# learner-shx/SVG-IR

Hardware: AMD Instinct MI355X
Metric: Gaussian-surfels/sec fwd+bwd @800x800 (1 view) (higher is better)
Workload: dtype f32; 1 GPU; cfg2: rgss path, P=200000 surfels, 800x800, SH degree 3, S=5, VS=0, fwd+bwd, one view per step per GPU (BASELINE.json configs[1] = cfg2 at N=1; configs[3] = cfg4, view r on rank r, at N>1); num_rendered=673008, parallelism=view-parallel x1, per_rank_cpus=not pinned

## Files before the change

svg-ir_amd/csrc/api.hip:

```cpp
#include <algorithm>
#include <cstdarg>
#include <cstdio>
#include <atomic>
#include <cstdlib>
#include <ctime>
#include <memory>
#include <mutex>
#include <string>
#include <vector>

#include "common.hpp"
#include "workload_history.hpp"

using namespace svgir;

namespace {

thread_local std::string g_err;
std::atomic<bool> g_prof{false};
WorkloadHistory g_history;
unsigned long long* pinned_words(size_t n) {
    void* ptr = nullptr;
    if (hipHostMalloc(&ptr, n * sizeof(unsigned long long), hipHostMallocCoherent) != hipSuccess) { (void)hipGetLastError(); return nullptr; }
    std::fill_n((unsigned long long*)ptr, n, 0ull);
    return (unsigned long long*)ptr;
}
unsigned long long* g_pinned = nullptr;
std::atomic<uint32_t> g_pinned_tag{0};
constexpr unsigned kPinnedSlots = 256;
std::once_flag g_pinned_once;
std::mutex g_pinned_mu;
uint64_t g_pinned_busy[kPinnedSlots / 64];
struct PinnedSlot {
    unsigned long long* at = nullptr; uint32_t tag = 0; int index = -1;
    PinnedSlot() {
        std::call_once(g_pinned_once, [] { g_pinned = pinned_words(2 * kPinnedSlots); });
        tag = ++g_pinned_tag;
        if (tag == 0) tag = ++g_pinned_tag;
        if (!g_pinned) return;
        static const unsigned usable = [] { const char* e = getenv("SVGIR_PINNED_SLOTS"); return e ? (unsigned)std::min<long>(std::max<long>(atol(e), 0), kPinnedSlots) : kPinnedSlots; }();
        std::lock_guard<std::mutex> lk(g_pinned_mu);
        for (unsigned i = 0; i < usable; i++)
            if (!(g_pinned_busy[i / 64] >> (i % 64) & 1ull)) {
                g_pinned_busy[i / 64] |= 1ull << (i % 64);
                index = (int)i;
                at = g_pinned + 2 * index;
                return;
            }
    }
    ~PinnedSlot() {
        if (index < 0) return;
        std::lock_guard<std::mutex> lk(g_pinned_mu);
        g_pinned_busy[index / 64] &= ~(1ull << (index % 64));
    }
    PinnedSlot(const PinnedSlot&) = delete;
    PinnedSlot& operator=(const PinnedSlot&) = delete;
};
double spin_budget_s() {
    static const double v = [] {
        const char* e = getenv("SVGIR_SPIN_MS");
        return e ? std::max(0.0, atof(e)) * 1e-3 : 0.05;
    }();
    return v;
}
// ... 252 lines not shown
        if (p->variant != SVGIR_SVGSS) return fail(SVGIR_ERR_INVALID, "fused shading belongs to the svgss variant");
        if (sp.P != p->P) return fail(SVGIR_ERR_INVALID, "fused shading: sp.P = %d but P = %d", sp.P, p->P);
        if (p->S != (sp.training ? 4 : 7) || p->VS != (sp.training ? 52 : 64))
            return fail(SVGIR_ERR_INVALID, "fused shading packs S = %d, VS = %d (training = %d), not S = %d, VS = %d", sp.training ? 4 : 7,
                        sp.training ? 52 : 64, sp.training, p->S, p->VS);
        if (!sp.viewmatrix) return fail(SVGIR_ERR_INVALID, "fused shading needs sp.viewmatrix (packed view-space normals)");
    }
    return 0;
}

CapKey workload_key(const svgir_params* p) {
    int dev_id = 0;
    (void)hipGetDevice(&dev_id);
    return CapKey{dev_id, p->W, p->H, p->P, p->S, p->variant == SVGIR_SVGSS ? p->VS : 0, p->variant, p->workload_scope};
}

bool bin_capacity(size_t bytes, const char* image_blob, int W, int H, int nstate, Wait how, const hipStream_t* stream, ViewCounts* vc) {
    const bool compact = bin_bytes_compact(bytes);
    if (compact || how != Wait::kCaps)
        *vc = resolve_view(image_blob, image_layout(const_cast<char*>(image_blob), W, H).counters, how, stream, compact);
    if (compact) return vc->known && vc->cap_slots >= 0;
    vc->cap_R = binning_capacity_from_bytes(bytes, view_grid(W, H).T, nstate);
    vc->cap_slots = -1;
    return true;
}

template <class A> void camera_args(A& a, const svgir_params* p) {
    a.P = p->P; a.D = p->D; a.M = p->M; a.means3D = p->means3D; a.shs = p->colors_precomp ? nullptr : p->shs;
    a.scales = p->scales; a.rotations = p->rotations; a.view = p->viewmatrix; a.proj = p->projmatrix; a.campos = p->cam_pos;
    a.scale_modifier = p->scale_modifier; a.tanx = p->tan_fovx; a.tany = p->tan_fovy; a.cfg = cfg_ref(p);
    a.focal_x = p->W / (2.0f * p->tan_fovx); a.focal_y = p->H / (2.0f * p->tan_fovy);
}

RenderArgs render_args(const svgir_params* p, const ViewGrid& v, const GeomLayout& G, const ImageLayout& I, const BinLayout& B, int fin) {
    const bool svgss = p->variant == SVGIR_SVGSS;
    RenderArgs ra{};
    ra.W = v.W; ra.H = v.H; ra.gx = v.gx; ra.gy = v.gy; ra.S = p->S; ra.VS = svgss ? p->VS : 0;
    ra.ranges = I.ranges; ra.point_list = B.val[fin]; ra.rec = G.rec; ra.features = p->features; ra.vfeatures = p->vfeatures;
    ra.bg = p->background; ra.cfg = cfg_ref(p);
    ra.sub_list = B.sub_list; ra.sub_total = I.sub_total; ra.sub_order = I.sub_order; ra.sub_count = I.sub_count; ra.sub_ndump = I.sub_ndump;
    ra.sub_pair_base = I.sub_pair_base; ra.sub_slot_base = I.sub_slot_base;
    ra.seg_list = B.seg_list; ra.seg_desc = B.seg_desc; ra.seg_count = I.counters; ra.seg_block = I.seg_block; ra.seg_state = B.seg_state;
    ra.slot_cap = (uint32_t)std::min<size_t>(B.slot_cap, 0xffffffffu);
    ra.order_n = (int)order_entries(v.gx, v.gy);
    ra.bg_in_render = render_specialised(p->S, ra.VS, svgss) ? 1 : 0;
    ra.final_T = I.final_T; ra.final_D = I.final_D; ra.n_contrib = I.n_contrib;
    return ra;
}
}

extern "C" {

int svgir_abi_version(void) { return SVGIR_ABI_VERSION; }
size_t svgir_geom_bytes(int32_t P) { return geom_layout(nullptr, P).bytes; }
size_t svgir_image_bytes(int32_t W, int32_t H) { return image_layout(nullptr, W, H).bytes; }
size_t svgir_binning_bytes(int32_t R, int32_t W, int32_t H, int32_t S, int32_t VS) {
    return bin_layout(nullptr, binning_capacity(R), view_grid(W, H).T, seg_nstate(S, VS)).bytes;
}
size_t svgir_image_ncontrib_offset(int32_t W, int32_t H) { return image_layout(nullptr, W, H).ncontrib_off; }
size_t svgir_image_ranges_offset(int32_t W, int32_t H) {
    const ImageLayout I = image_layout((char*)256, W, H);
    return (size_t)((char*)I.ranges - (char*)256);
}
size_t svgir_binning_point_list_offset(size_t binning_bytes, const char* image_blob, int32_t W, int32_t H, int32_t S, int32_t VS) {
    const int T = view_grid(W, H).T, nstate = seg_nstate(S, VS);
    ViewCounts vc;
    if (!bin_capacity(binning_bytes, image_blob, W, H, nstate, Wait::kCaps, nullptr, &vc)) return (size_t)-1;
    const BinLayout B = bin_layout((char*)256, vc.cap_R, T, nstate);
    return (size_t)((char*)B.val[tile_sort_plan(T).passes & 1] - (char*)256);
}
const char* svgir_last_error(void) { return g_err.c_str(); }
void svgir_set_profiling(int enabled) {
    resolve_pending();
    if (enabled) {
        std::lock_guard<std::mutex> lk(g_times_mu);
        g_accum.clear();
    }
    g_prof.store(enabled != 0);
}
int svgir_last_timings(const char** names, float* avg_ms, int* counts, int cap) {
    resolve_pending();
    std::lock_guard<std::mutex> lk(g_times_mu);
    int n = 0;
    for (auto& acc : g_accum) {
        if (n >= cap) break;
        names[n] = acc.name;
        avg_ms[n] = (float)(acc.sum_ms / (acc.count > 0 ? acc.count : 1));
        if (counts) counts[n] = acc.count;
        n++;
    }
    return n;
}

struct ForwardCall {
    const svgir_view_call c; const svgir_params* p = c.params; const svgir_outputs* o = c.outputs; hipStream_t s = (hipStream_t)c.stream;
    bool key_spec;
    int P = 0, nstate = 0, fin = 0, spec_top = -1, cap = 0;
    ViewGrid v{};
    bool svgss = false, shade_subset = false, prepass = false, done = false;
    char *gblob = nullptr, *iblob = nullptr, *bblob = nullptr;
    GeomLayout G{}; ImageLayout I{}; TileSortPlan plan{};
    CapKey ckey{}; const uint32_t* depth_order = nullptr; long long cap_slots = -1;
    hipEvent_t features_ready = nullptr;
    PinnedSlot R_pin;
    StageMarks tm;

    ForwardCall(const svgir_view_call& c_, bool key_spec_) : c(c_), key_spec(key_spec_), tm(stage_begin(s)) {}

    int check(const char* what) {
        hipError_t e = p->debug ? hipStreamSynchronize(s) : hipSuccess;
        if (e == hipSuccess) e = hipGetLastError();
        return e != hipSuccess ? fail(SVGIR_ERR_HIP, p->debug ? "%s failed: %s" : "%s launch failed: %s", what, hipGetErrorString(e)) : 0;
    }

    int run_binning_and_render(char* bblob, int cap, long long cap_slots, bool timed, bool cull_only = false) {
        const BinLayout B = bin_layout(bblob, cap, v.T, nstate, cap_slots);
        launch_emit(P, depth_order, G.tiles, G.offsets, G.rec, o->radii, v.gx, v.gy, B.key[0], B.val[0], cap, I.ranges,
                    I.counters, B.radix_tbl, G.counters + 3, s);
        if (int rc = check("emit")) return rc;
        if (timed) stage_mark(tm, "emit");
        if (plan.single) {
            launch_tile_sort12(B.key, B.val, cap, G.counters, B.radix_tbl, I.ranges, v.T, s);
            if (int rc = check("tile sort")) return rc;
            if (timed) stage_mark(tm, "sort_tile");
        } else {
            launch_radix_sort(B.key, B.val, cap, G.counters, plan.bits, plan.bits_per_pass, B.radix_tbl, s);
            if (int rc = check("tile sort")) return rc;
            if (timed) stage_mark(tm, "sort_tile");
            launch_ranges(cap, G.counters, B.key[fin], I.ranges, v.T, s);
            if (int rc = check("ranges")) return rc;
            if (timed) stage_mark(tm, "ranges");
        }

        RenderArgs ra = render_args(p, v, G, I, B, fin);
        ra.hi_fill = high_fill(g_history.guess_fill(ckey)) ? 1 : 0;
        ra.out_color = o->out_color; ra.out_normal = o->out_normal; ra.out_depth = o->out_depth; ra.out_opacity = o->out_opacity;
        ra.out_feature = o->out_feature; ra.out_vfeature = o->out_vfeature; ra.out_weights = o->out_weights;
        const bool clear_stencil = !svgss && !p->computer_pseudo_normal;
        ra.zero_a = clear_stencil ? o->out_pseudo_normal : nullptr;
        ra.zero_b = clear_stencil ? o->out_surface_xyz : nullptr;
        launch_cull(ra, s);
        uint32_t vtag = 0;
        unsigned long long* vslot = view_note(iblob, cap, cap_slots, &vtag, s);
        const bool row_path = svgss && p->VS > 0 && render_specialised(p->S, p->VS, true);
        static const int xcd_forced = [] { const char* e = getenv("SVGIR_FWD_XCD"); return e ? (atoi(e) != 0 ? 1 : 0) : -1; }();
        const bool per_xcd = ra.bg_in_render && (xcd_forced >= 0 ? xcd_forced != 0 : ra.hi_fill != 0);
        launch_order_desc(I.sub_total, 4 * v.T, I.sub_order, row_path ? I.sub_pair_base : nullptr, I.sub_slot_base, I.counters, vslot, vtag,
                          (uint32_t)cap, cap_slots, kBlobMagic, v.gx, ra.order_n, per_xcd, s);
        if (int rc = check("cull")) return rc;
        if (timed) stage_mark(tm, "cull");
        if (cull_only) return 0;
        if (prepass) {
            RenderArgs rp = ra;
            rp.S = 0; rp.VS = 0; rp.features = nullptr; rp.vfeatures = nullptr; rp.needed = G.needed;
            launch_contrib_prepass(rp, s);
            if (int rc = check("prepass")) return rc;
            if (timed) stage_mark(tm, "prepass");
        }
        if (p->shade) {
            svgir_shade_params sp = p->shade->sp;
            sp.subset = nullptr; sp.subset_count = nullptr;
            if (prepass) {
                uint32_t* cnt = G.shade_work + partition_work_words(P) - 1;
                launch_partition(P, G.needed, nullptr, G.shade_list, G.shade_work, cnt, s);
                sp.subset = G.shade_list; sp.subset_count = cnt;
            } else if (shade_subset) {
                sp.subset = depth_order; sp.subset_count = G.counters + 3;
            }
            if (shade_forward_impl(&sp, p->shade->reduced, const_cast<float*>(p->features), const_cast<float*>(p->vfeatures), true, s) != 0)
                return fail(SVGIR_ERR_INVALID, "fused shading: svgir_shade_forward rejected its parameters");
            if (int rc = check("shade")) return rc;
            if (timed) stage_mark(tm, "shade");
        }
        if (features_ready && hipStreamWaitEvent(s, features_ready, 0) != hipSuccess) return fail(SVGIR_ERR_HIP, "waiting for the features event");
        if (launch_render_fwd(ra, svgss, s) < 0) launch_render_fwd_generic(ra, svgss, s);
        if (int rc = check("render")) return rc;
        if (timed) stage_mark(tm, "render");
        return 0;
    }

    int begin() {
        if (int rc = validate(p, true)) return rc;
        features_ready = (hipEvent_t)p->features_ready;
        if (!o || !c.geom || !c.binning || !c.image) return fail(SVGIR_ERR_INVALID, "outputs / allocators must be provided");
        P = p->P; v = view_grid(p->W, p->H);
        svgss = p->variant == SVGIR_SVGSS;
        if (P == 0) {
            const size_t N = (size_t)v.W * v.H;
            HIP_OK(hipMemsetAsync(o->out_color, 0, 3 * N * 4, s));
            HIP_OK(hipMemsetAsync(o->out_normal, 0, 3 * N * 4, s));
            HIP_OK(hipMemsetAsync(o->out_depth, 0, N * 4, s));
            HIP_OK(hipMemsetAsync(o->out_opacity, 0, N * 4, s));
            if (p->S) HIP_OK(hipMemsetAsync(o->out_feature, 0, (size_t)p->S * N * 4, s));
            if (svgss && p->VS) HIP_OK(hipMemsetAsync(o->out_vfeature, 0, (size_t)(p->VS / 4) * N * 4, s));
            if (!svgss && o->out_pseudo_normal) HIP_OK(hipMemsetAsync(o->out_pseudo_normal, 0, 3 * N * 4, s));
            if (!svgss && o->out_surface_xyz) HIP_OK(hipMemsetAsync(o->out_surface_xyz, 0, 3 * N * 4, s));
            done = true;
            return 1;
        }
        gblob = c.geom(geom_layout(nullptr, P).bytes, c.geom_ctx);
        iblob = c.image(image_layout(nullptr, v.W, v.H).bytes, c.image_ctx);
        if (!gblob || !iblob) return fail(SVGIR_ERR_ALLOC, "geometry/image blob allocation failed");
        G = geom_layout(gblob, P);
        I = image_layout(iblob, v.W, v.H);

        PreArgs pa;
        camera_args(pa, p);
        pa.W = v.W; pa.H = v.H; pa.gx = v.gx; pa.gy = v.gy; pa.colors_precomp = p->colors_precomp; pa.opacities = p->opacities;
        pa.cov3D_precomp = p->cov3D_precomp; pa.patchbbox = p->patchbbox;
        pa.rec = G.rec; pa.cov3D = G.cov3D; pa.clamped = G.clamped; pa.tiles = G.tiles; pa.key = G.key[0]; pa.idx = G.idx[0];
        pa.radii = o->radii;
        pa.out_weights = o->out_weights;
        pa.features = nullptr; pa.embed_S = 0;
        if (rec_embeds_features(p->S, svgss ? p->VS : 0)) {
            if (features_ready && hipStreamWaitEvent(s, features_ready, 0) != hipSuccess) return fail(SVGIR_ERR_HIP, "waiting for the features event");
            features_ready = nullptr; pa.features = p->features; pa.embed_S = p->S; }
        shade_subset = p->shade && !p->shade->all_surfels;
        prepass = shade_subset && shade_prepass(p->shade->sp.Ns);
        pa.needed = prepass ? G.needed : nullptr;
        pa.span = G.counters + 3;
        if (p->shade) pa.tabs = shade_tables(&p->shade->sp, nullptr, 0);
        pa.zero_words = radix_gtot(G.radix_tbl, P); pa.n_zero_words = (int)radix_gtot_words(P);
        ckey = workload_key(p);
        static const bool key_spec_env = getenv("SVGIR_NO_KEY_SPEC") == nullptr;
        spec_top = (key_spec && key_spec_env) ? g_history.guess_top(ckey) : -1;
        pa.spec_top = spec_top; pa.key_top = G.key_top;
        pa.prefilter_violation = nullptr;
        if (p->prefiltered) {
            HIP_OK(hipMemsetAsync(G.counters, 0, 16, s));
            pa.prefilter_violation = G.counters + 1;
        }
        launch_preprocess(pa, svgss, s);
        if (int rc = check("preprocess")) return rc;
        stage_mark(tm, "preprocess");

        const int depth_bits = spec_top >= 0 ? 24 : 32;
        depth_order = G.idx[(depth_bits / 8) & 1];
        launch_radix_sort(G.key, G.idx, P, nullptr, depth_bits, 8, G.radix_tbl, s);
        if (int rc = check("depth sort")) return rc;
        stage_mark(tm, "sort_depth");

        launch_offsets_scan(G.tiles, depth_order, G.offsets, G.scan_tmp, P, G.counters, G.key_top, (P + 63) / 64, pa.prefilter_violation,
                            R_pin.at, R_pin.tag, s);
        if (int rc = check("offsets scan")) return rc;
        stage_mark(tm, "scan");

        nstate = seg_nstate(p->S, svgss ? p->VS : 0);
        plan = tile_sort_plan(v.T);
        fin = plan.passes & 1;

        cap = 0; cap_slots = -1; bblob = nullptr;
        CapKey pkey = ckey;
        (void)resolve_view(g_history.last_view(ckey, &pkey.P), nullptr, Wait::kLook, nullptr, false, &pkey);
        long long gs = -1;
        if (const int guess = g_history.guess(ckey, &gs)) {
            cap = binning_capacity((long long)guess + guess / 8 + 1024);
            cap_slots = p->forward_only ? 0 : (gs < 0 ? -1 : std::min<long long>(gs + gs / 8 + 64, (long long)seg_capacity(cap, v.T)));
            bblob = c.binning(bin_layout(nullptr, cap, v.T, nstate, cap_slots).bytes, c.binning_ctx);
            if (bblob) {
                if (int rc = run_binning_and_render(bblob, cap, cap_slots, true)) return rc;
            } else {
                cap = 0;
            }
        }
        return 0;
    }

    static int run(const svgir_view_call& c, bool key_spec) {
        ForwardCall f(c, key_spec);
        const int rc = f.begin();
        return rc != 0 ? (rc < 0 ? rc : 0) : f.finish();
    }

    int finish() {
        if (done) return 0;
        done = true;
        uint32_t R_host = 0, R_aux = 0;
        bool have_R = R_pin.at && pinned_spin(R_pin.at, R_pin.tag, &R_host, &R_aux);
        if (!have_R) {
            const hipError_t e = hipStreamSynchronize(s);
            if (e != hipSuccess) return fail(SVGIR_ERR_HIP, "the forward failed on the device: %s", hipGetErrorString(e));
            have_R = R_pin.at && tagged_pair(R_pin.at, R_pin.tag, &R_host, &R_aux);
            if (!have_R) {
                uint32_t w[3] = {0, 0, 0};
                HIP_OK(hipMemcpy(w, G.counters, 12, hipMemcpyDeviceToHost));
                R_host = w[0]; R_aux = ((p->prefiltered && w[1]) ? 1u << 16 : 0u) | (w[2] & 0xffffu);
            }
        }
        if (p->prefiltered && (R_aux >> 16) != 0u) {
            (void)hipStreamSynchronize(s);
            return fail(SVGIR_ERR_INVALID, "Point is filtered although prefiltered is set. This shouldn't happen!");
        }
        if (R_host > 0x7ffff000u) return fail(SVGIR_ERR_INVALID, "instance count %u overflows int32", R_host);
        const int R = (int)R_host;
        {
            const uint32_t summary = R_aux & 0xffffu;
            if (key_spec) { g_history.record_top(ckey, summary); g_history.count(WorkloadHistory::kForwards); }
            if (spec_top >= 0) g_history.count(WorkloadHistory::kThreePass);
            const int av = (int)((summary >> 8) & 0xffu), ov = (int)(summary & 0xffu);
            if (spec_top >= 0 && !(av == 0xff && ov == 0) && (av != spec_top || ov != spec_top)) {
                HIP_OK(hipStreamSynchronize(s));
                g_history.count(WorkloadHistory::kRerunTop);
// ... 345 lines not shown
```

svg-ir_amd/csrc/binning.hip:

```cpp
#include <algorithm>

#include "common.hpp"

namespace svgir {

namespace {

constexpr int GS = 32;

template <int ITEMS>
__global__ void __launch_bounds__(BLOCK) radix_hist_kernel(const uint32_t* __restrict__ keys, int n_cap,
                                                           const uint32_t* __restrict__ n_dev, int bit_lo,
                                                           uint32_t mask, uint32_t* __restrict__ table,
                                                           uint32_t* __restrict__ gtot) {
    __shared__ uint32_t hist[256];
    const int n = n_dev ? (int)min((uint32_t)n_cap, n_dev[0]) : n_cap;
    hist[threadIdx.x] = 0;
    __syncthreads();
    const int base = blockIdx.x * (BLOCK * ITEMS);
    uint32_t k[ITEMS];
#pragma unroll
    for (int i = 0; i < ITEMS; i++) k[i] = keys[max(0, min(base + i * BLOCK + (int)threadIdx.x, n - 1))];
#pragma unroll
    for (int i = 0; i < ITEMS; i++) {
        const int e = base + i * BLOCK + threadIdx.x;
        if (e < n) atomicAdd(&hist[(k[i] >> bit_lo) & mask], 1u);
    }
    __syncthreads();
    const uint32_t c = hist[threadIdx.x];
    table[(size_t)blockIdx.x * 256 + threadIdx.x] = c;
    if (c) atomicAdd(&gtot[(size_t)(blockIdx.x / GS) * 256 + threadIdx.x], c);
}

template <int ITEMS>
__global__ void __launch_bounds__(BLOCK) radix_scatter_kernel(const uint32_t* __restrict__ kin,
                                                              const uint32_t* __restrict__ vin,
                                                              uint32_t* __restrict__ kout, uint32_t* __restrict__ vout,
                                                              int n_cap, const uint32_t* __restrict__ n_dev, int bit_lo, int nbits,
                                                              const uint32_t* __restrict__ table,
                                                              const uint32_t* __restrict__ gtot, int ngroups) {
    __shared__ uint32_t wcnt[4][256];
    __shared__ uint32_t wtot[4];
    const int t = threadIdx.x, lane = t & 63, wave = t >> 6;
    const uint32_t mask = (1u << nbits) - 1;
    const int n = n_dev ? (int)min((uint32_t)n_cap, n_dev[0]) : n_cap;
    const int base = blockIdx.x * (BLOCK * ITEMS) + wave * (64 * ITEMS);
    const unsigned long long lt_mask = (lane == 0) ? 0ull : (~0ull >> (64 - lane));
    uint32_t ks[ITEMS], vs[ITEMS], rk[ITEMS];
#pragma unroll
    for (int c = 0; c < ITEMS; c++) {
        const int e = base + c * 64 + lane;
        ks[c] = e < n ? kin[e] : 0u;
        vs[c] = e < n ? vin[e] : 0u;
    }
#pragma unroll
// ... 46 lines not shown
        uint32_t incl = bc;
#pragma unroll
        for (int d = 1; d < 64; d <<= 1) {
            const uint32_t o = __shfl_up(incl, d);
            if (lane >= d) incl += o;
        }
        __syncthreads();
        if (lane == 63) wtot[wave] = incl;
        __syncthreads();
        uint32_t woff = 0;
#pragma unroll
        for (int w = 0; w < 4; w++) woff += w < wave ? wtot[w] : 0u;
        const uint32_t bs = woff + incl - bc;
        bstart[t] = bs; gcur[t] = cursor;
        wcnt[0][t] = bs; wcnt[1][t] = bs + c0; wcnt[2][t] = bs + c0 + c1; wcnt[3][t] = bs + c0 + c1 + c2;
        __syncthreads();
#pragma unroll
        for (int c = 0; c < ITEMS; c++) {
            if (base + c * 64 + lane < n) {
                const uint32_t lp = wcnt[wave][(ks[c] >> bit_lo) & mask] + rk[c];
                sK[lp] = ks[c]; sV[lp] = vs[c];
            }
        }
        __syncthreads();
        const int nblk = min(BLOCK * ITEMS, n - (int)blockIdx.x * (BLOCK * ITEMS));
#pragma unroll
        for (int c = 0; c < ITEMS; c++) {
            const int i = c * BLOCK + t;
            if (i < nblk) {
                const uint32_t k = sK[i], d = (k >> bit_lo) & mask;
                const uint32_t pos = gcur[d] + ((uint32_t)i - bstart[d]);
                kout[pos] = k;
                vout[pos] = sV[i];
            }
        }
        return;
    }
    {
        const uint32_t c0 = wcnt[0][t], c1 = wcnt[1][t], c2 = wcnt[2][t];
        __syncthreads();
        wcnt[0][t] = cursor; wcnt[1][t] = cursor + c0; wcnt[2][t] = cursor + c0 + c1; wcnt[3][t] = cursor + c0 + c1 + c2;
    }
    __syncthreads();
#pragma unroll
    for (int c = 0; c < ITEMS; c++) {
        if (base + c * 64 + lane < n) {
            const uint32_t pos = wcnt[wave][(ks[c] >> bit_lo) & mask] + rk[c];
            kout[pos] = ks[c];
            vout[pos] = vs[c];
        }
    }
}

__global__ void __launch_bounds__(BLOCK) ts12_hist_kernel(const uint32_t* __restrict__ keys, int n_cap, const uint32_t* __restrict__ n_dev,
                                                          uint32_t* __restrict__ table, int nbins) {
    __shared__ uint32_t hist[TS12_BINS];
    const int n = n_dev ? (int)min((uint32_t)n_cap, n_dev[0]) : n_cap;
    const int t = threadIdx.x;
    for (int i = t; i < nbins; i += BLOCK) hist[i] = 0u;
    __syncthreads();
    const int base = blockIdx.x * TS12_KEYS;
    uint32_t k[TS12_KEYS / BLOCK];
#pragma unroll
    for (int i = 0; i < TS12_KEYS / BLOCK; i++) k[i] = keys[max(0, min(base + i * BLOCK + t, n - 1))];
#pragma unroll
    for (int i = 0; i < TS12_KEYS / BLOCK; i++)
        if (base + i * BLOCK + t < n) atomicAdd(&hist[k[i] & (TS12_BINS - 1)], 1u);
    __syncthreads();
    uint32_t* row = table + (size_t)blockIdx.x * nbins;
    for (int i = t; i < nbins; i += BLOCK) row[i] = hist[i];
}

__global__ void __launch_bounds__(BLOCK) ts12_colscan_kernel(uint32_t* __restrict__ table, int nb, uint32_t* __restrict__ totals, int nbins) {
    __shared__ uint32_t psum[16][17];
    const int col = threadIdx.x & 15, seg = threadIdx.x >> 4;
    const int d = blockIdx.x * 16 + col;
    const int rps = (nb + 15) / 16, r0 = min(nb, seg * rps), r1 = min(nb, r0 + rps);
    uint32_t* colp = table + d;
    uint32_t sum = 0;
    int r = r0;
    for (; r + 8 <= r1; r += 8) {
        uint32_t c[8];
#pragma unroll
        for (int j = 0; j < 8; j++) c[j] = colp[(size_t)(r + j) * nbins];
#pragma unroll
        for (int j = 0; j < 8; j++) sum += c[j];
    }
    for (; r < r1; r++) sum += colp[(size_t)r * nbins];
    psum[seg][col] = sum;
    __syncthreads();
    uint32_t run = 0, all = 0;
#pragma unroll
    for (int sg = 0; sg < 16; sg++) { const uint32_t v = psum[sg][col]; run += sg < seg ? v : 0u; all += v; }
    if (seg == 0) totals[d] = all;
    r = r0;
    for (; r + 8 <= r1; r += 8) {
        uint32_t c[8];
#pragma unroll
        for (int j = 0; j < 8; j++) c[j] = colp[(size_t)(r + j) * nbins];
#pragma unroll
        for (int j = 0; j < 8; j++) { colp[(size_t)(r + j) * nbins] = run; run += c[j]; }
    }
    for (; r < r1; r++) { const uint32_t c = colp[(size_t)r * nbins]; colp[(size_t)r * nbins] = run; run += c; }
}

__global__ void __launch_bounds__(BLOCK) ts12_scatter_kernel(const uint32_t* __restrict__ kin, const uint32_t* __restrict__ vin,
                                                             uint32_t* __restrict__ kout, uint32_t* __restrict__ vout, int n_cap,
                                                             const uint32_t* __restrict__ n_dev, const uint32_t* __restrict__ table,
                                                             const uint32_t* __restrict__ totals, uint32_t* __restrict__ ranges, int T, int nbins) {
    __shared__ uint32_t cur[TS12_BINS];
    __shared__ uint16_t wcnt[4][TS12_BINS];
    __shared__ uint32_t wtot[4];
    constexpr int PERMAX = TS12_BINS / BLOCK;
    constexpr int ROUNDS = TS12_KEYS / BLOCK;
    const int per = nbins / BLOCK;
    const int t = threadIdx.x, lane = t & 63, wave = t >> 6;
    const int n = n_dev ? (int)min((uint32_t)n_cap, n_dev[0]) : n_cap;
    const int base = blockIdx.x * TS12_KEYS + wave * (64 * ROUNDS);
    const unsigned long long lt_mask = (lane == 0) ? 0ull : (~0ull >> (64 - lane));
    uint32_t ks[ROUNDS], vs[ROUNDS];
    uint16_t rk[ROUNDS];
#pragma unroll
    for (int c = 0; c < ROUNDS; c++) {
        const int e = base + c * 64 + lane;
        ks[c] = e < n ? kin[e] : 0u;
        vs[c] = e < n ? vin[e] : 0u;
    }
    uint32_t tot[PERMAX], pre[PERMAX];
    {
        const uint32_t* tp = totals + t * per;
        const uint32_t* rp = table + (size_t)blockIdx.x * nbins + t * per;
#pragma unroll
        for (int j = 0; j < PERMAX; j++) { tot[j] = j < per ? tp[j] : 0u; pre[j] = j < per ? rp[j] : 0u; }
    }
    uint32_t sum = 0;
#pragma unroll
    for (int j = 0; j < PERMAX; j++) sum += tot[j];
    uint32_t incl = sum;
#pragma unroll
    for (int d = 1; d < 64; d <<= 1) {
        const uint32_t o = __shfl_up(incl, d);
        if (lane >= d) incl += o;
    }
    if (lane == 63) wtot[wave] = incl;
#pragma unroll
    for (int w = 0; w < 4; w++)
        for (int i = t; i < nbins / 2; i += BLOCK) reinterpret_cast<uint32_t*>(&wcnt[w][0])[i] = 0u;
    __syncthreads();
    uint32_t run = incl - sum;
#pragma unroll
    for (int w = 0; w < 4; w++) run += w < wave ? wtot[w] : 0u;
#pragma unroll
    for (int j = 0; j < PERMAX; j++) {
        if (j < per) {
            const int tile = t * per + j;
            cur[tile] = run + pre[j];
            if (blockIdx.x == 0 && tile < T) {
                ranges[2 * tile] = tot[j] ? run : 0u;
                ranges[2 * tile + 1] = tot[j] ? run + tot[j] : 0u;
            }
            run += tot[j];
        }
    }
#pragma unroll
    for (int c = 0; c < ROUNDS; c++) {
        const bool valid = base + c * 64 + lane < n;
        const uint32_t d = ks[c] & (TS12_BINS - 1);
        unsigned long long same = __ballot(valid);
#pragma unroll
        for (int b = 0; b < 12; b++) {
            const unsigned long long m = __ballot((d >> b) & 1u);
            same &= ((d >> b) & 1u) ? m : ~m;
        }
        const uint32_t in_round = (uint32_t)__popcll(same & lt_mask);
        const uint32_t prior = wcnt[wave][d];
        rk[c] = (uint16_t)(prior + in_round);
        if (valid && in_round == 0) wcnt[wave][d] = (uint16_t)(prior + (uint32_t)__popcll(same));
    }
    __syncthreads();
#pragma unroll
    for (int c = 0; c < ROUNDS; c++) {
        if (base + c * 64 + lane < n) {
            const uint32_t d = ks[c] & (TS12_BINS - 1);
            uint32_t pos = cur[d] + rk[c];
            if (wave > 0) pos += wcnt[0][d];
            if (wave > 1) pos += wcnt[1][d];
            if (wave > 2) pos += wcnt[2][d];
            kout[pos] = ks[c];
            vout[pos] = vs[c];
        }
    }
}

__device__ __forceinline__ uint32_t block_exclusive_scan_2048(uint32_t (&v)[8], uint32_t* wsum, uint32_t& total) {
    const int t = threadIdx.x, lane = t & 63, wave = t >> 6;
    uint32_t s = 0;
#pragma unroll
    for (int i = 0; i < 8; i++) s += v[i];
    uint32_t incl = s;
#pragma unroll
    for (int d = 1; d < 64; d <<= 1) {
        const uint32_t o = __shfl_up(incl, d);
        if (lane >= d) incl += o;
    }
    if (lane == 63) wsum[wave] = incl;
    __syncthreads();
    uint32_t woff = 0, tot = 0;
#pragma unroll
    for (int w = 0; w < 4; w++) { const uint32_t x = wsum[w]; if (w < wave) woff += x; tot += x; }
    total = tot;
    return woff + incl - s;
}

__global__ void __launch_bounds__(BLOCK) offsets_reduce_kernel(const uint32_t* __restrict__ tiles,
                                                               const uint32_t* __restrict__ order, int n,
                                                               uint32_t* __restrict__ counts_out,
                                                               uint32_t* __restrict__ block_sums,
                                                               const uint32_t* __restrict__ key_top, int n_key_top,
                                                               uint32_t* __restrict__ block_key) {
    __shared__ uint32_t wsum[4];
    if (threadIdx.x < 64) {
        const int j = blockIdx.x * (SCAN_BLOCK_ELEMS / 64) + (int)threadIdx.x;
        uint32_t kv = (threadIdx.x < SCAN_BLOCK_ELEMS / 64 && j < n_key_top) ? key_top[j] : 0xff00u;
#pragma unroll
        for (int d = 32; d >= 1; d >>= 1) { const uint32_t o = (uint32_t)__shfl_xor((int)kv, d); kv = (kv & o & 0xff00u) | ((kv | o) & 0xffu); }
        if (threadIdx.x == 0) block_key[blockIdx.x] = kv;
    }
    uint32_t v[8];
    const int base = blockIdx.x * SCAN_BLOCK_ELEMS + threadIdx.x * 8;
    uint32_t oi[8];
#pragma unroll
    for (int i = 0; i < 8; i++) oi[i] = order[min(base + i, n - 1)];
#pragma unroll
    for (int i = 0; i < 8; i++) v[i] = tiles[2 * oi[i]];
#pragma unroll
    for (int i = 0; i < 8; i++) v[i] = (base + i < n) ? v[i] : 0u;
    if (base + 8 <= n) {
        reinterpret_cast<uint4*>(counts_out + base)[0] = make_uint4(v[0], v[1], v[2], v[3]);
        reinterpret_cast<uint4*>(counts_out + base)[1] = make_uint4(v[4], v[5], v[6], v[7]);
    } else {
#pragma unroll
        for (int i = 0; i < 8; i++) if (base + i < n) counts_out[base + i] = v[i];
    }
// ... 345 lines not shown

void launch_order_desc(const uint32_t* counts, int n, uint32_t* order, uint32_t* prefix, uint32_t* slot_prefix, uint32_t* totals,
                       unsigned long long* host_totals, uint32_t host_tag, uint32_t cap_R, long long cap_slots, uint32_t magic, int gx, int order_n,
                       bool per_xcd, hipStream_t s) {
    if (per_xcd) hipLaunchKernelGGL(order_xcd_kernel, dim3(8), dim3(1024), 0, s, counts, n, order, prefix, slot_prefix, totals, host_totals,
                                    host_tag, cap_R, cap_slots, magic, gx, order_n);
    else hipLaunchKernelGGL(order_desc_kernel, dim3(1), dim3(1024), 0, s, counts, n, order, prefix, slot_prefix, totals, host_totals,
                            host_tag, cap_R, cap_slots, magic, order_n);
}

template <int ITEMS>
static void radix_sort_impl(uint32_t* const key[2], uint32_t* const val[2], int n, const uint32_t* n_dev, int total_bits,
                            int bits_per_pass, uint32_t* tbl, uint32_t* gtot, hipStream_t s) {
    const int per = BLOCK * ITEMS;
    const int nb = (n + per - 1) / per;
    const int ng = (nb + GS - 1) / GS;
    const int passes = (total_bits + bits_per_pass - 1) / bits_per_pass;
    for (int p = 0; p < passes; p++) {
        const int lo = p * bits_per_pass, nbits = std::min(bits_per_pass, total_bits - lo);
        uint32_t* gt = gtot + (size_t)p * ng * 256;
        hipLaunchKernelGGL((radix_hist_kernel<ITEMS>), dim3(nb), dim3(BLOCK), 0, s, key[p & 1], n, n_dev, lo,
                           (1u << nbits) - 1, tbl, gt);
        hipLaunchKernelGGL((radix_scatter_kernel<ITEMS>), dim3(nb), dim3(BLOCK), 0, s, key[p & 1], val[p & 1],
                           key[(p + 1) & 1], val[(p + 1) & 1], n, n_dev, lo, nbits, tbl, gt, ng);
    }
}

void launch_radix_sort(uint32_t* const key[2], uint32_t* const val[2], int n, const uint32_t* n_dev, int total_bits,
                       int bits_per_pass, uint32_t* table, hipStream_t s) {
    if (n <= 0) return;
    uint32_t* gtot = radix_gtot(table, n);
    if (n <= (1 << 20)) radix_sort_impl<4>(key, val, n, n_dev, total_bits, bits_per_pass, table, gtot, s);
    else radix_sort_impl<16>(key, val, n, n_dev, total_bits, bits_per_pass, table, gtot, s);
}

void launch_offsets_scan(const uint32_t* tiles, const uint32_t* order, uint32_t* offsets, uint32_t* scan_tmp, int n,
                         uint32_t* total_out, const uint32_t* key_top, int n_key_top, const uint32_t* violation,
                         unsigned long long* host_out, uint32_t host_tag, hipStream_t s) {
    const int nb = scan_blocks(n);
    uint32_t* block_key = scan_tmp + nb + 1;
    hipLaunchKernelGGL(offsets_reduce_kernel, dim3(nb), dim3(BLOCK), 0, s, tiles, order, n, offsets, scan_tmp, key_top, n_key_top, block_key);
    hipLaunchKernelGGL(offsets_write_kernel, dim3(nb), dim3(BLOCK), 0, s, n, scan_tmp, offsets, nb,
                       total_out, block_key, violation, host_out, host_tag);
}

void launch_emit(int P, const uint32_t* order, const uint32_t* tiles, const uint32_t* offsets, float* rec,
                 const int32_t* radii, int gx, int gy, uint32_t* tile_keys, uint32_t* vals, int cap, uint32_t* ranges,
                 uint32_t* seg_count, uint32_t* sort_table, const uint32_t* span, hipStream_t s) {
    hipLaunchKernelGGL(emit_kernel, dim3((P + BLOCK - 1) / BLOCK), dim3(BLOCK), 0, s, P, order, tiles, offsets, rec,
                       radii, gx, gy, tile_keys, vals, (uint32_t)cap, ranges, 2 * gx * gy + (gx * gy + 255) / 256 * SEG_BLOCK_STRIDE, seg_count,
                       radix_gtot(sort_table, cap), (int)radix_gtot_words(cap), span);
}

void launch_tile_sort12(uint32_t* const key[2], uint32_t* const val[2], int n, const uint32_t* n_dev, uint32_t* table, uint32_t* ranges, int T,
                        hipStream_t s) {
    if (n <= 0) return;
    const int nb = (n + TS12_KEYS - 1) / TS12_KEYS;
    const int nbins = (T + BLOCK - 1) / BLOCK * BLOCK;
    uint32_t* totals = table + (size_t)nb * nbins;
    hipLaunchKernelGGL(ts12_hist_kernel, dim3(nb), dim3(BLOCK), 0, s, key[0], n, n_dev, table, nbins);
    hipLaunchKernelGGL(ts12_colscan_kernel, dim3(nbins / 16), dim3(BLOCK), 0, s, table, nb, totals, nbins);
    hipLaunchKernelGGL(ts12_scatter_kernel, dim3(nb), dim3(BLOCK), 0, s, key[0], val[0], key[1], val[1], n, n_dev, table, totals, ranges, T, nbins);
}

void launch_ranges(int R, const uint32_t* R_dev, const uint32_t* tile_keys, uint32_t* ranges, int T, hipStream_t s) {
    if (R > 0) hipLaunchKernelGGL(ranges_kernel, dim3((R + BLOCK - 1) / BLOCK), dim3(BLOCK), 0, s, R, R_dev, tile_keys, ranges);
}

}
```

Baseline: 543.8 million surfels/s.

## Replace emit plus tile counting sort with direct per-gaussian-row bin count and placement

For the single-pass tile-sort plan, the emit-keys then histogram/colscan/scatter pipeline is replaced. Tile histograms are now counted directly from gaussians in depth order, in rows of G gaussians, and a placement kernel writes point-list values straight into their sorted slots. This removes the intermediate key/value arrays, one global pass and the separate offsets scan. The offsets-scan totals and host readback are folded into the column-scan kernel. In exchange, tile instances are expanded twice with wave-level scans, and the geometry blob grows by a per-row bin table.

```diff
diff --git a/svg-ir_amd/csrc/api.hip b/svg-ir_amd/csrc/api.hip
--- a/svg-ir_amd/csrc/api.hip
+++ b/svg-ir_amd/csrc/api.hip
@@ -10,6 +10,7 @@
 #include <vector>
 
 #include "common.hpp"
+#include "bin_rows.hpp"
 #include "workload_history.hpp"
 
 using namespace svgir;
@@ -368,7 +369,7 @@
 extern "C" {
 
 int svgir_abi_version(void) { return SVGIR_ABI_VERSION; }
-size_t svgir_geom_bytes(int32_t P) { return geom_layout(nullptr, P).bytes; }
+size_t svgir_geom_bytes(int32_t P) { return geom_blob_bytes(P); }
 size_t svgir_image_bytes(int32_t W, int32_t H) { return image_layout(nullptr, W, H).bytes; }
 size_t svgir_binning_bytes(int32_t R, int32_t W, int32_t H, int32_t S, int32_t VS) {
     return bin_layout(nullptr, binning_capacity(R), view_grid(W, H).T, seg_nstate(S, VS)).bytes;
@@ -431,15 +432,15 @@
 
     int run_binning_and_render(char* bblob, int cap, long long cap_slots, bool timed, bool cull_only = false) {
         const BinLayout B = bin_layout(bblob, cap, v.T, nstate, cap_slots);
-        launch_emit(P, depth_order, G.tiles, G.offsets, G.rec, o->radii, v.gx, v.gy, B.key[0], B.val[0], cap, I.ranges,
-                    I.counters, B.radix_tbl, G.counters + 3, s);
-        if (int rc = check("emit")) return rc;
-        if (timed) stage_mark(tm, "emit");
         if (plan.single) {
-            launch_tile_sort12(B.key, B.val, cap, G.counters, B.radix_tbl, I.ranges, v.T, s);
-            if (int rc = check("tile sort")) return rc;
+            launch_bin_place(P, depth_order, G.tiles, G.rec, v.gx, v.gy, geom_bin_table(gblob, P), B.val[fin], cap, I.ranges, I.counters, G.counters + 3, s);
+            if (int rc = check("tile placement")) return rc;
             if (timed) stage_mark(tm, "sort_tile");
         } else {
+            launch_emit(P, depth_order, G.tiles, G.offsets, G.rec, o->radii, v.gx, v.gy, B.key[0], B.val[0], cap, I.ranges,
+                        I.counters, B.radix_tbl, G.counters + 3, s);
+            if (int rc = check("emit")) return rc;
+            if (timed) stage_mark(tm, "emit");
             launch_radix_sort(B.key, B.val, cap, G.counters, plan.bits, plan.bits_per_pass, B.radix_tbl, s);
             if (int rc = check("tile sort")) return rc;
             if (timed) stage_mark(tm, "sort_tile");
@@ -514,7 +515,7 @@
             done = true;
             return 1;
         }
-        gblob = c.geom(geom_layout(nullptr, P).bytes, c.geom_ctx);
+        gblob = c.geom(geom_blob_bytes(P), c.geom_ctx);
         iblob = c.image(image_layout(nullptr, v.W, v.H).bytes, c.image_ctx);
         if (!gblob || !iblob) return fail(SVGIR_ERR_ALLOC, "geometry/image blob allocation failed");
         G = geom_layout(gblob, P);
@@ -556,14 +557,18 @@
         if (int rc = check("depth sort")) return rc;
         stage_mark(tm, "sort_depth");
 
-        launch_offsets_scan(G.tiles, depth_order, G.offsets, G.scan_tmp, P, G.counters, G.key_top, (P + 63) / 64, pa.prefilter_violation,
-                            R_pin.at, R_pin.tag, s);
+        plan = tile_sort_plan(v.T);
+        fin = plan.passes & 1;
+        if (plan.single)
+            launch_bin_count(G.tiles, depth_order, P, v.gx, v.gy, geom_bin_table(gblob, P), G.counters, G.key_top, (P + 63) / 64, pa.prefilter_violation, R_pin.at,
+                             R_pin.tag, s);
+        else
+            launch_offsets_scan(G.tiles, depth_order, G.offsets, G.scan_tmp, P, G.counters, G.key_top, (P + 63) / 64, pa.prefilter_violation,
+                                R_pin.at, R_pin.tag, s);
         if (int rc = check("offsets scan")) return rc;
         stage_mark(tm, "scan");
 
         nstate = seg_nstate(p->S, svgss ? p->VS : 0);
-        plan = tile_sort_plan(v.T);
-        fin = plan.passes & 1;
 
         cap = 0; cap_slots = -1; bblob = nullptr;
         CapKey pkey = ckey;
diff --git a/svg-ir_amd/csrc/bin_rows.hpp b/svg-ir_amd/csrc/bin_rows.hpp
--- /dev/null
+++ b/svg-ir_amd/csrc/bin_rows.hpp
@@ -0,0 +1,33 @@
+#pragma once
+#include "common.hpp"
+
+namespace svgir {
+
+constexpr int BIN_G_MIN = 256, BIN_G_MAX = 32768, BIN_ROWS_MAX = 2048;
+inline int bin_row_gaussians(int P) {
+    static const int forced = [] { const char* e = getenv("SVGIR_BIN_G"); return e ? atoi(e) : 0; }();
+    int g = BIN_G_MIN;
+    while (g < BIN_G_MAX && g < forced) g *= 2;
+    while (g < BIN_G_MAX && ((P > 0 ? P : 1) + g - 1) / g > BIN_ROWS_MAX) g *= 2;
+    return g;
+}
+inline int bin_rows(int P) { const int g = bin_row_gaussians(P); return ((P > 0 ? P : 1) + g - 1) / g; }
+inline size_t bin_table_words(int P) { return ((size_t)bin_rows(P) + 1) * TS12_BINS + 2 * (size_t)bin_rows(P); }
+inline size_t geom_blob_bytes(int P) { return geom_layout(nullptr, P).bytes + align_up(bin_table_words(P) * 4); }
+inline uint32_t* geom_bin_table(char* geom_blob, int P) { return (uint32_t*)(geom_blob + geom_layout(nullptr, P).bytes); }
+struct BinRows { int G, rows, nbins; uint32_t *table, *totals, *row_sums, *row_key; };
+inline BinRows bin_rows_of(uint32_t* tbl, int P, int T) {
+    BinRows r;
+    r.G = bin_row_gaussians(P); r.rows = bin_rows(P); r.nbins = (T + BLOCK - 1) / BLOCK * BLOCK;
+    r.table = tbl; r.totals = tbl + (size_t)r.rows * r.nbins;
+    r.row_sums = tbl + ((size_t)r.rows + 1) * TS12_BINS; r.row_key = r.row_sums + r.rows;
+    return r;
+}
+
+void launch_bin_count(const uint32_t* tiles, const uint32_t* order, int P, int gx, int gy, uint32_t* bin_tbl, uint32_t* total_out,
+                      const uint32_t* key_top, int n_key_top, const uint32_t* violation, unsigned long long* host_out, uint32_t host_tag,
+                      hipStream_t s);
+void launch_bin_place(int P, const uint32_t* order, const uint32_t* tiles, float* rec, int gx, int gy, uint32_t* bin_tbl, uint32_t* vals,
+                      int cap, uint32_t* ranges, uint32_t* seg_count, const uint32_t* span, hipStream_t s);
+
+}
diff --git a/svg-ir_amd/csrc/binning.hip b/svg-ir_amd/csrc/binning.hip
--- a/svg-ir_amd/csrc/binning.hip
+++ b/svg-ir_amd/csrc/binning.hip
@@ -1,6 +1,6 @@
 #include <algorithm>
 
-#include "common.hpp"
+#include "bin_rows.hpp"
 
 namespace svgir {
 
@@ -153,27 +153,144 @@
     }
 }
 
-__global__ void __launch_bounds__(BLOCK) ts12_hist_kernel(const uint32_t* __restrict__ keys, int n_cap, const uint32_t* __restrict__ n_dev,
-                                                          uint32_t* __restrict__ table, int nbins) {
+
+__device__ __forceinline__ uint32_t wave_excl(uint32_t n, uint32_t& M) {
+    const int lane = threadIdx.x & 63;
+    uint32_t incl = n;
+#pragma unroll
+    for (int d = 1; d < 64; d <<= 1) {
+        const uint32_t o = (uint32_t)__shfl_up((int)incl, d);
+        if (lane >= d) incl += o;
+    }
+    M = (uint32_t)__builtin_amdgcn_readlane((int)incl, 63);
+    return incl - n;
+}
+
+__device__ __forceinline__ uint32_t wave_max_scan(uint32_t v) {
+    v = max(v, (uint32_t)__builtin_amdgcn_update_dpp(0, (int)v, 0x111, 0xf, 0xf, false));
+    v = max(v, (uint32_t)__builtin_amdgcn_update_dpp(0, (int)v, 0x112, 0xf, 0xf, false));
+    v = max(v, (uint32_t)__builtin_amdgcn_update_dpp(0, (int)v, 0x114, 0xf, 0xf, false));
+    v = max(v, (uint32_t)__builtin_amdgcn_update_dpp(0, (int)v, 0x118, 0xf, 0xf, false));
+    v = max(v, (uint32_t)__builtin_amdgcn_update_dpp(0, (int)v, 0x142, 0xa, 0xf, false));
+    v = max(v, (uint32_t)__builtin_amdgcn_update_dpp(0, (int)v, 0x143, 0xc, 0xf, false));
+    return v;
+}
+
+template <class F>
+__device__ __forceinline__ void wave_instances(uint32_t n, uint32_t loc, uint32_t M, uint32_t rect, uint32_t g, int gx, uint32_t* own, F&& f) {
+    const int lane = threadIdx.x & 63;
+    uint32_t carry = 1u;
+    for (uint32_t j0 = 0; j0 < M; j0 += 64u) {
+        const uint32_t j = j0 + (uint32_t)lane, rel = loc - j0;
+        own[lane] = 0u;
+        if (n != 0u && rel < 64u) own[rel] = (uint32_t)lane + 1u;
+        wave_lds_sync();
+        uint32_t v = own[lane];
+        wave_lds_sync();
+        v = max(wave_max_scan(v), carry);
+        carry = (uint32_t)__builtin_amdgcn_readlane((int)v, 63);
+        const int lo = (int)v - 1;
+        const uint32_t t = j - (uint32_t)__builtin_amdgcn_ds_bpermute(lo << 2, (int)loc);
+        const uint32_t go = (uint32_t)__builtin_amdgcn_ds_bpermute(lo << 2, (int)g);
+        const uint32_t ro = (uint32_t)__builtin_amdgcn_ds_bpermute(lo << 2, (int)rect);
+        const uint32_t w = max(ro >> 20, 1u), ty = t / w, tx = t - ty * w;
+        const bool live = j < M;
+        const uint32_t tile = ((((ro >> 10) & 1023u) + ty) * (uint32_t)gx + ((ro & 1023u) + tx)) & (uint32_t)(TS12_BINS - 1);
+        f(live, live ? tile : 0u, go);
+    }
+}
+
+template <class F>
+__device__ __forceinline__ void wave_tiles(uint32_t n, uint32_t loc, uint32_t M, uint32_t rect, uint32_t g, int gx, uint32_t* own, F&& f) {
+    const uint32_t nmax = (uint32_t)__builtin_amdgcn_readlane((int)wave_max_scan(n), 63);
+    if (nmax <= 64u) {
+        const uint32_t w = max(rect >> 20, 1u);
+        uint32_t row = ((rect >> 10) & 1023u) * (uint32_t)gx + (rect & 1023u), tx = 0;
+        for (uint32_t k = 0; k < nmax; k++) {
+            if (k < n) {
+                f((row + tx) & (uint32_t)(TS12_BINS - 1));
+                if (++tx == w) { tx = 0; row += (uint32_t)gx; }
+            }
+        }
+    } else {
+        wave_instances(n, loc, M, rect, g, gx, own, [&](bool live, uint32_t tile, uint32_t) { if (live) f(tile); });
+    }
+}
+
+__global__ void __launch_bounds__(BLOCK) bin_count_kernel(int P, int G, const uint32_t* __restrict__ order, const uint32_t* __restrict__ tiles,
+                                                          int gx, uint32_t* __restrict__ table, int nbins, uint32_t* __restrict__ row_sums,
+                                                          const uint32_t* __restrict__ key_top, int n_key_top, uint32_t* __restrict__ row_key,
+                                                          uint32_t* __restrict__ counters) {
     __shared__ uint32_t hist[TS12_BINS];
-    const int n = n_dev ? (int)min((uint32_t)n_cap, n_dev[0]) : n_cap;
-    const int t = threadIdx.x;
+    __shared__ uint32_t wsum[4], wkey[4], own[4][64];
+    const int t = threadIdx.x, lane = t & 63, wave = t >> 6;
+    const int quarter = G / 4, base = (int)blockIdx.x * G + wave * quarter;
+    const bool v0 = base + lane < P;
+    const uint32_t g0 = v0 ? order[base + lane] : 0u;
+    const uint2 tr0 = v0 ? reinterpret_cast<const uint2*>(tiles)[g0] : make_uint2(0u, 0u);
     for (int i = t; i < nbins; i += BLOCK) hist[i] = 0u;
-    __syncthreads();
-    const int base = blockIdx.x * TS12_KEYS;
-    uint32_t k[TS12_KEYS / BLOCK];
-#pragma unroll
-    for (int i = 0; i < TS12_KEYS / BLOCK; i++) k[i] = keys[max(0, min(base + i * BLOCK + t, n - 1))];
-#pragma unroll
-    for (int i = 0; i < TS12_KEYS / BLOCK; i++)
-        if (base + i * BLOCK + t < n) atomicAdd(&hist[k[i] & (TS12_BINS - 1)], 1u);
+    {
+        const int per = G / 64;
+        uint32_t kv = 0xff00u;
+        for (int j = t; j < per; j += BLOCK) {
+            const int e = (int)blockIdx.x * per + j;
+            const uint32_t x = e < n_key_top ? key_top[e] : 0xff00u;
+            kv = (kv & x & 0xff00u) | ((kv | x) & 0xffu);
+        }
+#pragma unroll
+        for (int d = 32; d >= 1; d >>= 1) { const uint32_t o = (uint32_t)__shfl_xor((int)kv, d); kv = (kv & o & 0xff00u) | ((kv | o) & 0xffu); }
+        if (lane == 0) wkey[wave] = kv;
+    }
+    __syncthreads();
+    uint32_t wtot = 0, span = 0;
+    for (int c = 0; c < quarter && base + c < P; c += 64) {
+        const int i = base + c + lane;
+        uint32_t g = g0;
+        uint2 tr = tr0;
+        if (c != 0) {
+            g = i < P ? order[i] : 0u;
+            tr = i < P ? reinterpret_cast<const uint2*>(tiles)[g] : make_uint2(0u, 0u);
+        }
+        if (tr.x != 0u) span = (uint32_t)(i + 1);
+        uint32_t M;
+        const uint32_t loc = wave_excl(tr.x, M);
+        wave_tiles(tr.x, loc, M, tr.y, g, gx, own[wave], [&](uint32_t tile) { atomicAdd(&hist[tile], 1u); });
+        wtot += M;
+    }
+#pragma unroll
+    for (int d = 32; d >= 1; d >>= 1) span = max(span, (uint32_t)__shfl_xor((int)span, d));
+    if (lane == 0) {
+        wsum[wave] = wtot;
+        if (span != 0u) atomicMax(counters + 3, span);
+    }
     __syncthreads();
     uint32_t* row = table + (size_t)blockIdx.x * nbins;
     for (int i = t; i < nbins; i += BLOCK) row[i] = hist[i];
-}
-
-__global__ void __launch_bounds__(BLOCK) ts12_colscan_kernel(uint32_t* __restrict__ table, int nb, uint32_t* __restrict__ totals, int nbins) {
+    if (t == 0) {
+        row_sums[blockIdx.x] = wsum[0] + wsum[1] + wsum[2] + wsum[3];
+        row_key[blockIdx.x] = (wkey[0] & wkey[1] & wkey[2] & wkey[3] & 0xff00u) | ((wkey[0] | wkey[1] | wkey[2] | wkey[3]) & 0xffu);
+    }
+}
+
+__global__ void __launch_bounds__(BLOCK) ts12_colscan_kernel(uint32_t* __restrict__ table, int nrows, int G, const uint32_t* __restrict__ span,
+                                                             uint32_t* __restrict__ totals, int nbins, const uint32_t* __restrict__ row_sums,
+                                                             const uint32_t* __restrict__ row_key, uint32_t* __restrict__ total_out,
+                                                             const uint32_t* __restrict__ violation, unsigned long long* __restrict__ host_out,
+                                                             uint32_t host_tag) {
     __shared__ uint32_t psum[16][17];
+    __shared__ uint32_t rsum[4], ksum[4];
+    if (blockIdx.x == 0) {
+        uint32_t R = 0, kv = 0xff00u;
+        for (int r = threadIdx.x; r < nrows; r += BLOCK) { R += row_sums[r]; const uint32_t x = row_key[r]; kv = (kv & x & 0xff00u) | ((kv | x) & 0xffu); }
+#pragma unroll
+        for (int d = 32; d >= 1; d >>= 1) {
+            R += __shfl_xor(R, d);
+            const uint32_t o = (uint32_t)__shfl_xor((int)kv, d);
+            kv = (kv & o & 0xff00u) | ((kv | o) & 0xffu);
+        }
+        if ((threadIdx.x & 63) == 0) { rsum[threadIdx.x >> 6] = R; ksum[threadIdx.x >> 6] = kv; }
+    }
+    const int nb = min(nrows, (int)((span[0] + (uint32_t)G - 1u) / (uint32_t)G));
     const int col = threadIdx.x & 15, seg = threadIdx.x >> 4;
     const int d = blockIdx.x * 16 + col;
     const int rps = (nb + 15) / 16, r0 = min(nb, seg * rps), r1 = min(nb, r0 + rps);
@@ -190,6 +307,17 @@
     for (; r < r1; r++) sum += colp[(size_t)r * nbins];
     psum[seg][col] = sum;
     __syncthreads();
+    if (blockIdx.x == 0 && threadIdx.x == 0) {
+        const uint32_t R = rsum[0] + rsum[1] + rsum[2] + rsum[3];
+        const uint32_t summary = (ksum[0] & ksum[1] & ksum[2] & ksum[3] & 0xff00u) | ((ksum[0] | ksum[1] | ksum[2] | ksum[3]) & 0xffu);
+        total_out[0] = R;
+        total_out[2] = summary;
+        if (host_out) {
+            const uint32_t viol = violation ? (violation[0] != 0u ? 1u : 0u) : 0u;
+            __hip_atomic_store(host_out, ((unsigned long long)host_tag << 32) | R, __ATOMIC_RELAXED, __HIP_MEMORY_SCOPE_SYSTEM);
+            __hip_atomic_store(host_out + 1, ((unsigned long long)host_tag << 32) | (viol << 16) | summary, __ATOMIC_RELAXED, __HIP_MEMORY_SCOPE_SYSTEM);
+        }
+    }
     uint32_t run = 0, all = 0;
 #pragma unroll
     for (int sg = 0; sg < 16; sg++) { const uint32_t v = psum[sg][col]; run += sg < seg ? v : 0u; all += v; }
@@ -205,28 +333,31 @@
     for (; r < r1; r++) { const uint32_t c = colp[(size_t)r * nbins]; colp[(size_t)r * nbins] = run; run += c; }
 }
 
-__global__ void __launch_bounds__(BLOCK) ts12_scatter_kernel(const uint32_t* __restrict__ kin, const uint32_t* __restrict__ vin,
-                                                             uint32_t* __restrict__ kout, uint32_t* __restrict__ vout, int n_cap,
-                                                             const uint32_t* __restrict__ n_dev, const uint32_t* __restrict__ table,
-                                                             const uint32_t* __restrict__ totals, uint32_t* __restrict__ ranges, int T, int nbins) {
+__global__ void __launch_bounds__(BLOCK) bin_place_kernel(int P, int G, const uint32_t* __restrict__ order, const uint32_t* __restrict__ tiles,
+                                                          float* __restrict__ rec, int gx, int nbits, const uint32_t* __restrict__ table,
+                                                          const uint32_t* __restrict__ totals, const uint32_t* __restrict__ row_sums,
+                                                          uint32_t* __restrict__ ranges, int T, int nbins, uint32_t* __restrict__ vout, uint32_t cap,
+                                                          const uint32_t* __restrict__ span, uint32_t* __restrict__ seg_block, int n_seg_block,
+                                                          uint32_t* __restrict__ seg_count) {
     __shared__ uint32_t cur[TS12_BINS];
-    __shared__ uint16_t wcnt[4][TS12_BINS];
-    __shared__ uint32_t wtot[4];
+    __shared__ uint32_t wcnt[4][TS12_BINS / 2];
+    __shared__ uint32_t wtot[4], psum[4], wins[4], own[4][64];
     constexpr int PERMAX = TS12_BINS / BLOCK;
-    constexpr int ROUNDS = TS12_KEYS / BLOCK;
     const int per = nbins / BLOCK;
     const int t = threadIdx.x, lane = t & 63, wave = t >> 6;
-    const int n = n_dev ? (int)min((uint32_t)n_cap, n_dev[0]) : n_cap;
-    const int base = blockIdx.x * TS12_KEYS + wave * (64 * ROUNDS);
+    for (int j = (int)blockIdx.x * BLOCK + t; j < n_seg_block; j += (int)gridDim.x * BLOCK) seg_block[j] = 0u;
+    if (blockIdx.x == 0 && t == 0) seg_count[0] = 0u;
+    const int nvis = (int)min((uint32_t)P, span[0]);
+    if (blockIdx.x != 0 && (int)blockIdx.x * G >= nvis) return;
+    const int quarter = G / 4, base = (int)blockIdx.x * G + wave * quarter;
     const unsigned long long lt_mask = (lane == 0) ? 0ull : (~0ull >> (64 - lane));
-    uint32_t ks[ROUNDS], vs[ROUNDS];
-    uint16_t rk[ROUNDS];
-#pragma unroll
-    for (int c = 0; c < ROUNDS; c++) {
-        const int e = base + c * 64 + lane;
-        ks[c] = e < n ? kin[e] : 0u;
-        vs[c] = e < n ? vin[e] : 0u;
-    }
+    const bool v0 = base + lane < nvis;
+    const uint32_t g0 = v0 ? order[base + lane] : 0u;
+    const uint2 tr0 = v0 ? reinterpret_cast<const uint2*>(tiles)[g0] : make_uint2(0u, 0u);
+    uint32_t before = 0;
+    for (int b = t; b < (int)blockIdx.x; b += BLOCK) before += row_sums[b];
+#pragma unroll
+    for (int d = 32; d >= 1; d >>= 1) before += __shfl_xor(before, d);
     uint32_t tot[PERMAX], pre[PERMAX];
     {
         const uint32_t* tp = totals + t * per;
@@ -244,10 +375,12 @@
         if (lane >= d) incl += o;
     }
     if (lane == 63) wtot[wave] = incl;
+    if (lane == 0) psum[wave] = before;
 #pragma unroll
     for (int w = 0; w < 4; w++)
-        for (int i = t; i < nbins / 2; i += BLOCK) reinterpret_cast<uint32_t*>(&wcnt[w][0])[i] = 0u;
-    __syncthreads();
+        for (int i = t; i < nbins / 2; i += BLOCK) wcnt[w][i] = 0u;
+    __syncthreads();
+    before = psum[0] + psum[1] + psum[2] + psum[3];
     uint32_t run = incl - sum;
 #pragma unroll
     for (int w = 0; w < 4; w++) run += w < wave ? wtot[w] : 0u;
@@ -257,39 +390,66 @@
             const int tile = t * per + j;
             cur[tile] = run + pre[j];
             if (blockIdx.x == 0 && tile < T) {
-                ranges[2 * tile] = tot[j] ? run : 0u;
-                ranges[2 * tile + 1] = tot[j] ? run + tot[j] : 0u;
+                ranges[2 * tile] = tot[j] ? min(run, cap) : 0u;
+                ranges[2 * tile + 1] = tot[j] ? min(run + tot[j], cap) : 0u;
             }
             run += tot[j];
         }
     }
-#pragma unroll
-    for (int c = 0; c < ROUNDS; c++) {
-        const bool valid = base + c * 64 + lane < n;
-        const uint32_t d = ks[c] & (TS12_BINS - 1);
-        unsigned long long same = __ballot(valid);
-#pragma unroll
-        for (int b = 0; b < 12; b++) {
-            const unsigned long long m = __ballot((d >> b) & 1u);
-            same &= ((d >> b) & 1u) ? m : ~m;
-        }
-        const uint32_t in_round = (uint32_t)__popcll(same & lt_mask);
-        const uint32_t prior = wcnt[wave][d];
-        rk[c] = (uint16_t)(prior + in_round);
-        if (valid && in_round == 0) wcnt[wave][d] = (uint16_t)(prior + (uint32_t)__popcll(same));
-    }
-    __syncthreads();
-#pragma unroll
-    for (int c = 0; c < ROUNDS; c++) {
-        if (base + c * 64 + lane < n) {
-            const uint32_t d = ks[c] & (TS12_BINS - 1);
-            uint32_t pos = cur[d] + rk[c];
-            if (wave > 0) pos += wcnt[0][d];
-            if (wave > 1) pos += wcnt[1][d];
-            if (wave > 2) pos += wcnt[2][d];
-            kout[pos] = ks[c];
-            vout[pos] = vs[c];
-        }
+    uint32_t mine = 0;
+    for (int c = 0; c < quarter && base + c < nvis; c += 64) {
+        const int i = base + c + lane;
+        uint32_t g = g0;
+        uint2 tr = tr0;
+        if (c != 0) {
+            g = i < nvis ? order[i] : 0u;
+            tr = i < nvis ? reinterpret_cast<const uint2*>(tiles)[g] : make_uint2(0u, 0u);
+        }
+        uint32_t M;
+        const uint32_t loc = wave_excl(tr.x, M);
+        wave_tiles(tr.x, loc, M, tr.y, g, gx, own[wave], [&](uint32_t tile) { atomicAdd(&wcnt[wave][tile >> 1], 1u << ((tile & 1u) * 16u)); });
+        mine += M;
+    }
+    if (lane == 0) wins[wave] = mine;
+    __syncthreads();
+    for (int i = t; i < nbins / 2; i += BLOCK) {
+        const uint32_t c0 = wcnt[0][i], c1 = wcnt[1][i], c2 = wcnt[2][i];
+        wcnt[0][i] = 0u; wcnt[1][i] = c0; wcnt[2][i] = c0 + c1; wcnt[3][i] = c0 + c1 + c2;
+    }
+    __syncthreads();
+    uint32_t ibase = before;
+#pragma unroll
+    for (int w = 0; w < 4; w++) ibase += w < wave ? wins[w] : 0u;
+    uint16_t* const myc = reinterpret_cast<uint16_t*>(&wcnt[wave][0]);
+    for (int c = 0; c < quarter && base + c < nvis; c += 64) {
+        const int i = base + c + lane;
+        uint32_t g = g0;
+        uint2 tr = tr0;
+        if (c != 0) {
+            g = i < nvis ? order[i] : 0u;
+            tr = i < nvis ? reinterpret_cast<const uint2*>(tiles)[g] : make_uint2(0u, 0u);
+        }
+        uint32_t M;
+        const uint32_t loc = wave_excl(tr.x, M);
+        if (tr.x != 0u) {
+            rec[(size_t)g * REC + R_IBASE] = __builtin_bit_cast(float, ibase + loc);
+            rec[(size_t)g * REC + R_RECT] = __builtin_bit_cast(float, tr.y);
+        }
+        wave_instances(tr.x, loc, M, tr.y, g, gx, own[wave], [&](bool live, uint32_t d, uint32_t go) {
+            unsigned long long same = __ballot(live);
+            for (int b = 0; b < nbits; b++) {
+                const unsigned long long m = __ballot((d >> b) & 1u);
+                same &= ((d >> b) & 1u) ? m : ~m;
+            }
+            const uint32_t in_round = (uint32_t)__popcll(same & lt_mask);
+            const uint32_t prior = myc[d];
+            if (live) {
+                const uint32_t pos = cur[d] + prior + in_round;
+                if (pos < cap) vout[pos] = go;
+                if (in_round == 0) myc[d] = (uint16_t)(prior + (uint32_t)__popcll(same));
+            }
+        });
+        ibase += M;
     }
 }
 
@@ -741,15 +901,22 @@
                        radix_gtot(sort_table, cap), (int)radix_gtot_words(cap), span);
 }
 
-void launch_tile_sort12(uint32_t* const key[2], uint32_t* const val[2], int n, const uint32_t* n_dev, uint32_t* table, uint32_t* ranges, int T,
-                        hipStream_t s) {
-    if (n <= 0) return;
-    const int nb = (n + TS12_KEYS - 1) / TS12_KEYS;
-    const int nbins = (T + BLOCK - 1) / BLOCK * BLOCK;
-    uint32_t* totals = table + (size_t)nb * nbins;
-    hipLaunchKernelGGL(ts12_hist_kernel, dim3(nb), dim3(BLOCK), 0, s, key[0], n, n_dev, table, nbins);
-    hipLaunchKernelGGL(ts12_colscan_kernel, dim3(nbins / 16), dim3(BLOCK), 0, s, table, nb, totals, nbins);
-    hipLaunchKernelGGL(ts12_scatter_kernel, dim3(nb), dim3(BLOCK), 0, s, key[0], val[0], key[1], val[1], n, n_dev, table, totals, ranges, T, nbins);
+void launch_bin_count(const uint32_t* tiles, const uint32_t* order, int P, int gx, int gy, uint32_t* bin_tbl, uint32_t* total_out,
+                      const uint32_t* key_top, int n_key_top, const uint32_t* violation, unsigned long long* host_out, uint32_t host_tag,
+                      hipStream_t s) {
+    const BinRows r = bin_rows_of(bin_tbl, P, gx * gy);
+    hipLaunchKernelGGL(bin_count_kernel, dim3(r.rows), dim3(BLOCK), 0, s, P, r.G, order, tiles, gx, r.table, r.nbins, r.row_sums, key_top, n_key_top,
+                       r.row_key, total_out);
+    hipLaunchKernelGGL(ts12_colscan_kernel, dim3(r.nbins / 16), dim3(BLOCK), 0, s, r.table, r.rows, r.G, total_out + 3, r.totals, r.nbins, r.row_sums,
+                       r.row_key, total_out, violation, host_out, host_tag);
+}
+
+void launch_bin_place(int P, const uint32_t* order, const uint32_t* tiles, float* rec, int gx, int gy, uint32_t* bin_tbl, uint32_t* vals,
+                      int cap, uint32_t* ranges, uint32_t* seg_count, const uint32_t* span, hipStream_t s) {
+    const int T = gx * gy;
+    const BinRows r = bin_rows_of(bin_tbl, P, T);
+    hipLaunchKernelGGL(bin_place_kernel, dim3(r.rows), dim3(BLOCK), 0, s, P, r.G, order, tiles, rec, gx, tile_sort_plan(T).bits, r.table, r.totals,
+                       r.row_sums, ranges, T, r.nbins, vals, (uint32_t)cap, span, ranges + 2 * T, (T + 255) / 256 * SEG_BLOCK_STRIDE, seg_count);
 }
 
 void launch_ranges(int R, const uint32_t* R_dev, const uint32_t* tile_keys, uint32_t* ranges, int T, hipStream_t s) {
```

Result: no change. 539.2 million surfels/s (-0.8%).
